# sungnyun/dualhyp

Hardware: AMD Instinct MI355X
Metric: corrected utterances/sec (TinyLlama-1.1B, 5+5 hyps, 512->64 tok) (higher is better)
Workload: dtype bf16; 1 GPU; DualHyp inference, TinyLlama-1.1B bf16 + LoRA r16 (q,k,v,proj), batch 32/GPU synthetic 5+5-hyp prompts, 512-token prompt -> 64 generated tokens, greedy; batch_per_gpu=32, parallelism=replicas x1, batches_in_flight_per_gpu=64, schedule=merged, decode_rows_per_launch=2048

## Files before the change

### dualhyp_amd/csrc/capi.hip

```cpp
#include "common.h"
#include "tuning.h"
#include <stdarg.h>

static thread_local char g_err[512] = "";

void dh_set_error(const char* fmt, ...) {
    va_list ap;
    va_start(ap, fmt);
    vsnprintf(g_err, sizeof(g_err), fmt, ap);
    va_end(ap);
}

extern "C" const char* dh_last_error(void) { return g_err; }
extern "C" int dh_abi_version(void) { return DH_ABI_VERSION; }

int dh_stop_pack(const char* name, const dh_stop_spec* stop, bool start_ok, dh_stop_args& out) {
    out = dh_stop_args{};
    if (!stop) return 0;
    DH_CHECK(stop->n_seqs >= 0 && stop->n_seqs <= DH_MAX_STOP_SEQS, "%s: %d stop sequences, at most %d are supported", name, stop->n_seqs,
             DH_MAX_STOP_SEQS);
    DH_CHECK(stop->n_seqs == 0 || (stop->seqs && stop->h_seq_len), "%s: %d stop sequences without their ids or their lengths", name,
             stop->n_seqs);
    uint32_t lens = 0;
    for (int i = 0; i < stop->n_seqs; ++i) {
// ... 10 lines not shown
    return 0;
}

int dh_nucleus_pack(const char* name, float top_p, float min_p, dh_nucleus_args& out) {
    out = dh_nucleus_args{};
    DH_CHECK(top_p > 0.f && top_p <= 1.f, "%s: top_p=%g is not in (0, 1] (1 = off)", name, (double)top_p);
    DH_CHECK(min_p >= 0.f && min_p <= 1.f, "%s: min_p=%g is not in [0, 1] (0 = off)", name, (double)min_p);
    out.top_p = top_p;
    out.min_p = min_p;
    out.min_p_on = min_p > 0.f;
    out.lmin = out.min_p_on ? (float)log((double)min_p) : 0.f;
    return 0;
}

int dh_penalty_pack(const char* name, const dh_penalty_args* in, dh_penalty_args& out) {
    out = DH_PENALTY_OFF;
    if (!in) return 0;
    DH_CHECK(in->repetition >= 0.125f && in->repetition <= 8.f, "%s: repetition=%g is not in [1/8, 8] (1 = off)", name, (double)in->repetition);
    DH_CHECK(in->frequency >= -8.f && in->frequency <= 8.f, "%s: frequency=%g is not in [-8, 8] (0 = off)", name, (double)in->frequency);
    DH_CHECK(in->presence >= -8.f && in->presence <= 8.f, "%s: presence=%g is not in [-8, 8] (0 = off)", name, (double)in->presence);
    out = *in;
    return 0;
}

extern "C" int dh_device_info(char* h_buf, int h_buf_len, int* h_num_cu, int64_t* h_hbm_bytes) {
    int n = 0;
    hipError_t e = hipGetDeviceCount(&n);
    DH_CHECK(e == hipSuccess && n > 0, "no HIP device visible (%s)", hipGetErrorString(e));
    int dev = 0;
    DH_HIP(hipGetDevice(&dev));
    hipDeviceProp_t p;
    DH_HIP(hipGetDeviceProperties(&p, dev));
    if (h_buf && h_buf_len > 0) {
        strncpy(h_buf, p.gcnArchName, h_buf_len - 1);
        h_buf[h_buf_len - 1] = 0;
    }
    if (h_num_cu) *h_num_cu = p.multiProcessorCount;
    if (h_hbm_bytes) *h_hbm_bytes = (int64_t)p.totalGlobalMem;
    return 0;
}

namespace {

enum Accept { ANY, BOOL , RANGE , ONE_OF  };
struct TuningRow { int key; int* knob; Accept accept; int a, b, c; };
constexpr int NO_MAX = 0x7fffffff;

const TuningRow TUNING[] = {
    {0, &g_skinny_variant, ANY, 0, 0, 0},
    {1, &g_gemm_variant, ANY, 0, 0, 0},
    {2, &g_swiglu2, ANY, 0, 0, 0},
    {3, &g_mid, ANY, 0, 0, 0},
    {4, &g_linear_phase, ANY, 0, 0, 0},
    {5, &g_gemm_gm, RANGE, 0, NO_MAX, 0},
    {6, &g_dt_min_rows, RANGE, 1, NO_MAX, 0},
    {7, &g_chain_min_rows, RANGE, 1, NO_MAX, 0},
    {8, &g_dt_stages, ANY, 0, 0, 0},
    {9, &g_gemm128_stages, ANY, 0, 0, 0},
    {10, &g_decode_tiled_rows, RANGE, 0, NO_MAX, 0},
    {11, &g_rows_ct, RANGE, 0, NO_MAX, 0},
    {12, &g_fuse_qkv_rope, ANY, 0, 0, 0},
    {13, &g_mid_wlds, ANY, 0, 0, 0},
    {14, &g_rows_ng, ONE_OF, 0, 8, 10},
    {15, &g_dt_wide, ANY, 0, 0, 0},
    {16, &g_short_kps, ONE_OF, 8, 16, 16},
    {17, &g_pairs_wn, ONE_OF, 0, 2, 4},
    {18, &g_pairs_min_rows, RANGE, 1, NO_MAX, 0},
    {19, &g_fp8_tile, ONE_OF, 0, 128, 256},
    {20, &g_fp8_gm, RANGE, 0, 64, 0},
    {21, &g_pairs_wt, BOOL, 0, 0, 0},
    {22, &g_w4_persist, RANGE, 0, 2, 0},
    {23, &g_prune_last_layer, BOOL, 0, 0, 0},
    {24, &g_w4_fast_epi, ANY, 0, 0, 0},
    {25, &g_w4_persist_qkv, BOOL, 0, 0, 0},
    {26, &g_tn_mfma, BOOL, 0, 0, 0},
    {27, &g_attn_bwd_dq_group, BOOL, 0, 0, 0},
    {28, &g_tail_split, BOOL, 0, 0, 0},
    {29, &g_attn_bwd_dkdv_img, BOOL, 0, 0, 0},
    {30, &g_w4_persist_lora, BOOL, 0, 0, 0},
    {31, &g_skinny_n, BOOL, 0, 0, 0},
    {40, &g_attn_chain, BOOL, 0, 0, 0},
    {41, &g_finish_hoist_rows, RANGE, -1, NO_MAX, 0},
    {42, &g_prefill_wpb, ONE_OF, 0, 2, 4},
};

}

extern "C" int dh_set_tuning(int key, int value) {
    for (const TuningRow& r : TUNING) {
        if (r.key != key) continue;
        if (r.accept == RANGE && (value < r.a || value > r.b)) break;
        if (r.accept == ONE_OF && value != r.a && value != r.b && value != r.c) break;
        *r.knob = r.accept == BOOL ? value != 0 : value;
        return 0;
    }
    dh_set_error("dh_set_tuning: unknown key %d", key);
    return 1;
}
```

### dualhyp_amd/csrc/decode_fused.hip

```cpp
#include "common.h"
#include "tuning.h"

int g_attn_chain = 1;
int g_finish_hoist_rows = -1;

#ifdef DH_ATTN_STAMPS
__device__ unsigned long long g_attn_stamps[4096 * 8];
#define ATTN_STAMP(i) do { if (threadIdx.x == 0 && blockIdx.x < 4096) g_attn_stamps[blockIdx.x * 8 + (i)] = __builtin_amdgcn_s_memrealtime(); } while (0)
#define ATTN_DRAIN() __builtin_amdgcn_s_waitcnt(0)
extern "C" int dh_debug_attn_stamps(unsigned long long* out) {
    return hipMemcpyFromSymbol(out, HIP_SYMBOL(g_attn_stamps), sizeof(g_attn_stamps)) == hipSuccess ? 0 : 1;
}
#else
#define ATTN_STAMP(i)
#define ATTN_DRAIN()
#endif

namespace {

constexpr int DCOLS = 16;
constexpr int MAXP = 16;

template <int HS, int PMAX, int NW>
__global__ __launch_bounds__(NW * 64, NW == 16 ? 1 : (NW == 6 ? 3 : (HS == 64 ? 4 : 2))) void attn_decode_fused_kernel(
    const float* __restrict__ qkv32, int n_part, int pairs, int n_seq, int ldq, int qkv_dim,
    const bf16_t* __restrict__ lora_b, float lora_scale, int split0, int split1,
    const bf16_t* __restrict__ cos, const bf16_t* __restrict__ sin, const int32_t* __restrict__ seq_slot,
    const int32_t* __restrict__ kv_len, bf16_t* __restrict__ k_cache, bf16_t* __restrict__ vT_cache,
    bf16_t* __restrict__ y, int n_head, int n_groups, int s_max, float scale) {
    constexpr int KS = HS / 16, DT = HS / 32, HALF = HS / 2;
    extern __shared__ __attribute__((aligned(16))) char smem[];
    const int pair = blockIdx.x, seq = pair / n_groups, g = pair % n_groups;
    const int q_per_kv = n_head / n_groups;
    const int tid = threadIdx.x, lane = tid & 63, wave = tid >> 6;
    const int lr = lane & 31, lh = lane >> 5;
    const int slot = seq_slot[seq];
    const int len = kv_len[seq], pos = len - 1;
    bf16_t* sQ = reinterpret_cast<bf16_t*>(smem);
    float* sKn = reinterpret_cast<float*>(smem + 16 * HS * 2);
    float* sVn = sKn + HS;
    float* sXa = sVn + HS;
    float* sSn = sXa + 48;
    float* sPm = sSn + 16;
    float* sPl = sPm + NW * DCOLS;
    float* sPo = sPl + NW * DCOLS;
    constexpr int NT_ = NW * 64;
    ATTN_STAMP(0);

    constexpr int PF = NW == 6 ? 2 : 1;
    struct VF { bf16x8 v; };
    struct Tile { bf16x8 kf[KS]; VF vf[DT][2]; };
    Tile tl[PF];
    const bf16_t* kbase = k_cache + ((size_t)slot * n_groups + g) * s_max * HS;
    const bf16_t* vbase = vT_cache + ((size_t)slot * n_groups + g) * HS * s_max;
    const int n_tiles = (pos + 31) / 32;
    auto load_tile = [&](Tile& T, int t) {
#pragma unroll
        for (int ks = 0; ks < KS; ++ks)
            T.kf[ks] = __builtin_nontemporal_load(reinterpret_cast<const bf16x8*>(kbase + kfrag_blk<HS>(t, ks) + lane * 8));
#pragma unroll
        for (int dt = 0; dt < DT; ++dt)
#pragma unroll
            for (int s2 = 0; s2 < 2; ++s2)
                T.vf[dt][s2].v = __builtin_nontemporal_load(reinterpret_cast<const bf16x8*>(vbase + vfrag_blk<HS>(t, dt, s2) + lane * 8));
    };
#pragma unroll
    for (int p = 0; p < PF; ++p)
        if (wave + NW * p < n_tiles) load_tile(tl[p], wave + NW * p);

    const float* row0 = qkv32 + (size_t)seq * ldq;
    const size_t pstride = (size_t)n_seq * ldq;
    auto psum = [&](int c) {
        float v[PMAX];
#pragma unroll
        for (int p = 0; p < PMAX; ++p) v[p] = p < n_part ? row0[p * pstride + c] : 0.f;
        float s = 0.f;
        if (pairs) {
#pragma unroll
            for (int p = 0; p < PMAX; p += 2) s += v[p] + v[p + 1];
        } else {
#pragma unroll
            for (int p = 0; p < PMAX; ++p) s += v[p];
        }
        return s;
    };
    if (lora_b != nullptr && tid < 48) sXa[tid] = rbf(psum(qkv_dim + tid));
    for (int i = tid; i < 16 * HS; i += NT_) sQ[i] = 0;
// ... 698 lines not shown
        const int c0 = (tid + i * 256) * 8;
        if (c0 < d) {
            float acc[8];
#pragma unroll
            for (int e = 0; e < 8; ++e) acc[e] = 0.f;
            for (int p0 = 0; p0 < n_part; p0 += 4) {
                float4 a0[4], a1[4];
#pragma unroll
                for (int q = 0; q < 4; ++q) {
                    if (HOIST && i == 0 && p0 == 0) {
                        a0[q] = ha0[q]; a1[q] = ha1[q];
                        continue;
                    }
                    const int p = p0 + q < n_part ? p0 + q : p0;
                    a0[q] = *reinterpret_cast<const float4*>(hrow + p * pstride + c0);
                    a1[q] = *reinterpret_cast<const float4*>(hrow + p * pstride + c0 + 4);
                }
                if (pairs) {
#pragma unroll
                    for (int q = 0; q < 4; q += 2) {
                        if (p0 + q < n_part) {
                            const bool two = p0 + q + 1 < n_part;
                            const float4 b0 = two ? a0[q + 1] : float4{0.f, 0.f, 0.f, 0.f}, b1 = two ? a1[q + 1] : float4{0.f, 0.f, 0.f, 0.f};
                            acc[0] += a0[q].x + b0.x; acc[1] += a0[q].y + b0.y; acc[2] += a0[q].z + b0.z; acc[3] += a0[q].w + b0.w;
                            acc[4] += a1[q].x + b1.x; acc[5] += a1[q].y + b1.y; acc[6] += a1[q].z + b1.z; acc[7] += a1[q].w + b1.w;
                        }
                    }
                } else {
#pragma unroll
                for (int q = 0; q < 4; ++q) {
                    if (p0 + q < n_part) {
                        acc[0] += a0[q].x; acc[1] += a0[q].y; acc[2] += a0[q].z; acc[3] += a0[q].w;
                        acc[4] += a1[q].x; acc[5] += a1[q].y; acc[6] += a1[q].z; acc[7] += a1[q].w;
                    }
                }
                }
            }
            const uint4 xr = HOIST && i == 0 ? hxr : *reinterpret_cast<const uint4*>(x_resid + (size_t)row * d + c0);
            const bf16_t* xp = reinterpret_cast<const bf16_t*>(&xr);
            uint4 xo;
            bf16_t* xop = reinterpret_cast<bf16_t*>(&xo);
#pragma unroll
            for (int e = 0; e < 8; ++e) {
                float o = rbf(acc[e]);
                if (lora_b != nullptr) {
                    const uint4* b4 = reinterpret_cast<const uint4*>(lora_b + (size_t)(c0 + e) * 16);
                    float l = 0.f;
#pragma unroll
                    for (int h = 0; h < 2; ++h) {
                        const uint4 bv = b4[h];
                        const bf16_t* bp = reinterpret_cast<const bf16_t*>(&bv);
#pragma unroll
                        for (int k = 0; k < 8; ++k) l = fmaf(sXa[h * 8 + k], bf2f(bp[k]), l);
                    }
                    o = rbf(o + rbf(rbf(l) * lora_scale));
                }
                xop[e] = f2bf(bf2f(xp[e]) + o);
                v[i][e] = bf2f(xop[e]);
                ss += rbf(v[i][e] * v[i][e]);
            }
            *reinterpret_cast<uint4*>(x_out + (size_t)row * d + c0) = xo;
        }
    }
    ss = wave_sum(ss);
    if (lane == 0) sRed[wave] = ss;
    __syncthreads();
    ss = sRed[0] + sRed[1] + sRed[2] + sRed[3];
    const float ms = rbf(ss / (float)d);
    const float t = rbf(ms + eps);
    const bool tail = row_tail != nullptr && row_tail[row] != 0;
    const float r = tail ? rbf(1.0f / rbf(sqrtf(t))) : rbf(1.0f / sqrtf(t));
#pragma unroll
    for (int i = 0; i < MAXC; ++i) {
        const int c0 = (tid + i * 256) * 8;
        if (c0 < d) {
            const uint4 wu = HOIST && i == 0 ? hwu : *reinterpret_cast<const uint4*>(w_norm + c0);
            const bf16_t* wp = reinterpret_cast<const bf16_t*>(&wu);
            uint4 o;
            bf16_t* op = reinterpret_cast<bf16_t*>(&o);
#pragma unroll
            for (int e = 0; e < 8; ++e) op[e] = f2bf(bf2f(wp[e]) * rbf(v[i][e] * r));
            *reinterpret_cast<uint4*>(xn_out + (size_t)row * d + c0) = o;
        }
    }
}

}

extern "C" int dh_attn_decode_fused_bf16(const float* qkv32, int n_part, int pairs, int n_seq, int qkv_dim, int n_ext,
                                         const dh_bf16* lora_b, float lora_scale, int split0, int split1,
                                         const dh_bf16* cos, const dh_bf16* sin, const int32_t* seq_slot,
                                         const int32_t* kv_len, dh_bf16* k_cache, dh_bf16* vT_cache, dh_bf16* y,
                                         int n_head, int n_groups, int hs, int s_max, void* stream) {
    DH_CHECK(qkv32 && cos && sin && seq_slot && kv_len && k_cache && vT_cache && y, "dh_attn_decode_fused_bf16: null argument");
    DH_CHECK(n_groups > 0 && n_head % n_groups == 0 && n_head / n_groups <= DCOLS, "dh_attn_decode_fused_bf16: bad head counts");
    DH_CHECK(hs == 64 || hs == 96 || hs == 128, "dh_attn_decode_fused_bf16: head_size %d unsupported", hs);
    DH_CHECK(s_max % 64 == 0 && n_part >= 1 && n_part <= MAXP, "dh_attn_decode_fused_bf16: bad s_max / n_part");
    DH_CHECK(qkv_dim == (n_head + 2 * n_groups) * hs, "dh_attn_decode_fused_bf16: qkv_dim mismatch");
    DH_CHECK(lora_b == nullptr || n_ext >= 48, "dh_attn_decode_fused_bf16: LoRA needs the 48 x·A^T columns");
    if (n_seq <= 0) return 0;
    const float scale = 1.0f / sqrtf((float)hs);
    hipStream_t s = (hipStream_t)stream;
    dim3 grid(n_seq * n_groups);
#define ATT_LAUNCH(HSV, PM)                                                                                           \
    hipLaunchKernelGGL((attn_decode_fused_kernel<HSV, PM, attn_fused_waves<HSV>()>), grid, dim3(64 * attn_fused_waves<HSV>()), attn_fused_lds<HSV>(), s, qkv32, n_part, pairs, n_seq,  \
                       qkv_dim + n_ext, qkv_dim, lora_b, lora_scale, split0, split1, cos, sin, seq_slot, kv_len, k_cache,  \
                       vT_cache, y, n_head, n_groups, s_max, scale)
#define CHAIN_LAUNCH(PM)                                                                                              \
    hipLaunchKernelGGL((attn_decode_chain_kernel<64, PM, CHAIN_NW>), grid, dim3(64 * CHAIN_NW), attn_chain_lds<64>(), s, qkv32, n_part, pairs, n_seq,  \
                       qkv_dim + n_ext, qkv_dim, lora_b, lora_scale, split0, split1, cos, sin, seq_slot, kv_len, k_cache,  \
                       vT_cache, y, n_head, n_groups, s_max, scale)
    if (hs == 64) {
        DH_MAX_LDS_ONCE((attn_decode_fused_kernel<64, 2, attn_fused_waves<64>()>), attn_fused_lds<64>());
        DH_MAX_LDS_ONCE((attn_decode_fused_kernel<64, 8, attn_fused_waves<64>()>), attn_fused_lds<64>());
        DH_MAX_LDS_ONCE((attn_decode_fused_kernel<64, 16, attn_fused_waves<64>()>), attn_fused_lds<64>());
        const bool chain = g_attn_chain != 0 && attn_fused_waves<64>() == CHAIN_NW && (n_head / n_groups + 1) * 32 + 64 <= 64 * CHAIN_NW;
        if (chain) {
            DH_MAX_LDS_ONCE((attn_decode_chain_kernel<64, 2, CHAIN_NW>), attn_chain_lds<64>());
            DH_MAX_LDS_ONCE((attn_decode_chain_kernel<64, 8, CHAIN_NW>), attn_chain_lds<64>());
            DH_MAX_LDS_ONCE((attn_decode_chain_kernel<64, 16, CHAIN_NW>), attn_chain_lds<64>());
            if (n_part <= 2) CHAIN_LAUNCH(2);
            else if (n_part <= 8) CHAIN_LAUNCH(8);
            else CHAIN_LAUNCH(16);
        } else if (n_part <= 2) ATT_LAUNCH(64, 2);
        else if (n_part <= 8) ATT_LAUNCH(64, 8);
        else ATT_LAUNCH(64, 16);
    } else if (hs == 96) {
        DH_MAX_LDS_ONCE((attn_decode_fused_kernel<96, 2, 8>), attn_fused_lds<96>());
        DH_MAX_LDS_ONCE((attn_decode_fused_kernel<96, 8, 8>), attn_fused_lds<96>());
        DH_MAX_LDS_ONCE((attn_decode_fused_kernel<96, 16, 8>), attn_fused_lds<96>());
        if (n_part <= 2) ATT_LAUNCH(96, 2);
        else if (n_part <= 8) ATT_LAUNCH(96, 8);
        else ATT_LAUNCH(96, 16);
    } else {
        DH_MAX_LDS_ONCE((attn_decode_fused_kernel<128, 2, 8>), attn_fused_lds<128>());
        DH_MAX_LDS_ONCE((attn_decode_fused_kernel<128, 8, 8>), attn_fused_lds<128>());
        DH_MAX_LDS_ONCE((attn_decode_fused_kernel<128, 16, 8>), attn_fused_lds<128>());
        if (n_part <= 2) ATT_LAUNCH(128, 2);
        else if (n_part <= 8) ATT_LAUNCH(128, 8);
        else ATT_LAUNCH(128, 16);
    }
#undef ATT_LAUNCH
#undef CHAIN_LAUNCH
    DH_LAUNCH_CHECK();
    return 0;
}

int dh_attn_verify_fused_impl(const float* qkv32, int n_part, int pairs, int n_seq, int S, int qkv_dim, int n_ext,
                              const dh_bf16* lora_b, float lora_scale, int split0, int split1, const dh_bf16* cos,
                              const dh_bf16* sin, const int32_t* seq_slot, const int32_t* kv_len, dh_bf16* k_cache,
                              dh_bf16* vT_cache, dh_bf16* y, int n_head, int n_groups, int hs, int s_max, int p_max, void* stream) {
    DH_CHECK(qkv32 && cos && sin && seq_slot && kv_len && k_cache && vT_cache && y, "attn_verify_fused: null argument");
    DH_CHECK(n_groups > 0 && n_head % n_groups == 0, "attn_verify_fused: bad head counts");
    DH_CHECK(S >= 2 && S <= 8, "attn_verify_fused: S = %d positions per sequence, 2 .. 8 are served", S);
    DH_CHECK(S * (n_head / n_groups) <= 32, "attn_verify_fused: %d positions x %d heads per group exceed 32 query columns",
             S, n_head / n_groups);
    DH_CHECK(hs == 64 || hs == 96 || hs == 128, "attn_verify_fused: head_size %d unsupported", hs);
    DH_CHECK(s_max % 64 == 0 && p_max > 0 && p_max <= s_max && n_part >= 1 && n_part <= MAXP, "attn_verify_fused: bad s_max / p_max / n_part");
    DH_CHECK(qkv_dim == (n_head + 2 * n_groups) * hs, "attn_verify_fused: qkv_dim mismatch");
    DH_CHECK(lora_b == nullptr || n_ext >= 48, "attn_verify_fused: LoRA needs the 48 x·A^T columns");
    if (n_seq <= 0) return 0;
    const float scale = 1.0f / sqrtf((float)hs);
    hipStream_t s = (hipStream_t)stream;
    dim3 grid(n_seq * n_groups);
    const int ncol = S * (n_head / n_groups);
#define VER_LAUNCH(HSV, PM)                                                                                           \
    hipLaunchKernelGGL((attn_verify_fused_kernel<HSV, PM, attn_fused_waves<HSV>()>), grid, dim3(64 * attn_fused_waves<HSV>()), attn_verify_lds<HSV>(S, ncol), s, qkv32, n_part, pairs, \
                       n_seq * S, qkv_dim + n_ext, qkv_dim, lora_b, lora_scale, split0, split1, cos, sin, seq_slot, kv_len, k_cache,  \
                       vT_cache, y, n_head, n_groups, s_max, p_max, S, scale)
#define VER_HS(HSV)                                                                                                   \
    do {                                                                                                              \
        DH_MAX_LDS_ONCE((attn_verify_fused_kernel<HSV, 2, attn_fused_waves<HSV>()>), attn_verify_lds<HSV>(8, 32));    \
        DH_MAX_LDS_ONCE((attn_verify_fused_kernel<HSV, 8, attn_fused_waves<HSV>()>), attn_verify_lds<HSV>(8, 32));    \
        DH_MAX_LDS_ONCE((attn_verify_fused_kernel<HSV, 16, attn_fused_waves<HSV>()>), attn_verify_lds<HSV>(8, 32));   \
        if (n_part <= 2) VER_LAUNCH(HSV, 2);                                                                          \
        else if (n_part <= 8) VER_LAUNCH(HSV, 8);                                                                     \
        else VER_LAUNCH(HSV, 16);                                                                                     \
    } while (0)
    if (hs == 64) VER_HS(64);
    else if (hs == 96) VER_HS(96);
    else VER_HS(128);
#undef VER_HS
#undef VER_LAUNCH
    DH_LAUNCH_CHECK();
    return 0;
}

extern "C" int dh_attn_verify_fused_bf16(const float* qkv32, int n_part, int pairs, int n_seq, int S, int qkv_dim, int n_ext,
                                         const dh_bf16* lora_b, float lora_scale, int split0, int split1, const dh_bf16* cos,
                                         const dh_bf16* sin, const int32_t* seq_slot, const int32_t* kv_len, dh_bf16* k_cache,
                                         dh_bf16* vT_cache, dh_bf16* y, int n_head, int n_groups, int hs, int s_max, int p_max,
                                         void* stream) {
    return dh_attn_verify_fused_impl(qkv32, n_part, pairs, n_seq, S, qkv_dim, n_ext, lora_b, lora_scale, split0, split1, cos, sin,
                                     seq_slot, kv_len, k_cache, vT_cache, y, n_head, n_groups, hs, s_max, p_max, stream);
}

constexpr int FINISH_HOIST_ROWS = 128;

extern "C" int dh_finish_norm_bf16(const float* h32, int n_part, int pairs, int rows, int d, int n_ext, const dh_bf16* lora_b,
                                   float lora_scale, const dh_bf16* x_resid, const dh_bf16* w_norm, dh_bf16* x_out,
                                   dh_bf16* xn_out, float eps, const uint8_t* row_tail, void* stream) {
    DH_CHECK(h32 && x_resid && w_norm && x_out && xn_out, "dh_finish_norm_bf16: null argument");
    DH_CHECK(d % 8 == 0 && d <= 8192 && n_part >= 1 && n_part <= MAXP, "dh_finish_norm_bf16: unsupported d=%d", d);
    DH_CHECK(lora_b == nullptr || n_ext >= 16, "dh_finish_norm_bf16: LoRA needs the 16 x·A^T columns");
    DH_CHECK((d + n_ext) % 4 == 0, "dh_finish_norm_bf16: row stride must be a multiple of 4 floats");
    if (rows <= 0) return 0;
    hipStream_t s = (hipStream_t)stream;
    dim3 grid(rows), block(256);
    const int ldh = d + n_ext;
#define LAUNCH(MAXC) do {                                                                                             \
        if (hoist) hipLaunchKernelGGL((finish_norm_kernel<MAXC, true>), grid, block, 0, s, h32, n_part, pairs, rows, ldh, lora_b,  \
                                      lora_scale, x_resid, w_norm, x_out, xn_out, d, eps, row_tail);                  \
        else hipLaunchKernelGGL((finish_norm_kernel<MAXC, false>), grid, block, 0, s, h32, n_part, pairs, rows, ldh, lora_b,       \
                                lora_scale, x_resid, w_norm, x_out, xn_out, d, eps, row_tail);                        \
    } while (0)
    const int hoist_rows = g_finish_hoist_rows >= 0 ? g_finish_hoist_rows : FINISH_HOIST_ROWS;
    const bool hoist = hoist_rows > 0 && rows >= hoist_rows;
    if (d <= 2048) { LAUNCH(1); }
    else if (d <= 4096) { LAUNCH(2); }
    else { LAUNCH(4); }
#undef LAUNCH
    DH_LAUNCH_CHECK();
    return 0;
}
```

### dualhyp_amd/csrc/gemm_dt.hip

```cpp
#include "common.h"
#include "gemm.h"

int g_dt_stages = 0;
int g_dt_wide = 0;

namespace {

constexpr int TB = 128;
constexpr int BKD = 64;
template <int WN> constexpr int stage_bytes() { return (WN * 64 + TB) * BKD * 2; }

__device__ __forceinline__ int swz7(int row) { return (row >> 1) & 7; }

struct DtArgs {
    const bf16_t* x;
    const bf16_t* w;
    const bf16_t* w2;
    void* y;
    const bf16_t* vec_a;
    const bf16_t* vec_b;
    const bf16_t* resid;
    int M, N, K, n_main, seg;
    int split_kt;
    int wt;
};

template <int MODE, int NSTAGE, int WN = 2>
__global__ __launch_bounds__(WN * 128) void gemm_dt_kernel(DtArgs a) {
    constexpr int STAGE = stage_bytes<WN>();
    constexpr int ASZ = WN * 64 * BKD * 2;
    constexpr int NB = 16 / (2 * WN);
    constexpr int PER = 4 + NB;
    extern __shared__ __attribute__((aligned(16))) char smem[];
    const int tid = threadIdx.x, lane = tid & 63, wave = tid >> 6;
    const int wn = wave >> 1, wm = wave & 1;
    const int frow = lane & 15, kg = lane >> 4;
    const int m_tiles = (a.M + TB - 1) / TB;
    int tile, ky = 0;
    {
        const int nwg = gridDim.x * gridDim.y, bid = blockIdx.x + gridDim.x * blockIdx.y, xcd = bid & 7, q = nwg >> 3, r = nwg & 7;
        tile = (xcd < r ? xcd * (q + 1) : r * (q + 1) + (xcd - r) * q) + (bid >> 3);
        if (MODE == 4) { ky = tile / (int)gridDim.x; tile -= ky * (int)gridDim.x; }
    }
    const int tm = tile % m_tiles, tn = tile / m_tiles;
    const int m0 = tm * TB;
    const int n0 = MODE == 1 ? tn * (WN * 32) : tn * (WN * 64);

    const bf16_t* srcA[4];
    const bf16_t* srcB[NB];
#pragma unroll
    for (int j = 0; j < 4; ++j) {
        const int R = wave * 4 + j;
        const int row = R * 8 + (lane >> 3);
        const int chunk = (lane & 7) ^ swz7(row);
        const bf16_t* base = a.w;
        int n;
        if (MODE == 1) {
            const int half = (row >> 5) & 1;
            n = n0 + (row >> 6) * 32 + (row & 31);
            n = n < a.N ? n : a.N - 1;
            base = half ? a.w2 : a.w;
        } else {
            n = n0 + row;
            n = n < a.N ? n : a.N - 1;
            if ((MODE == 0 || MODE == 4) && n >= a.n_main) { base = a.w2; n -= a.n_main; }
        }
        srcA[j] = base + (size_t)n * a.K + chunk * 8 + (MODE == 4 ? (size_t)ky * a.split_kt * BKD : 0);
    }
#pragma unroll
    for (int j = 0; j < NB; ++j) {
        const int R = wave * NB + j;
        const int row = R * 8 + (lane >> 3);
        const int chunk = (lane & 7) ^ swz7(row);
        int m = m0 + row;
        m = m < a.M ? m : a.M - 1;
        srcB[j] = a.x + (size_t)m * a.K + chunk * 8 + (MODE == 4 ? (size_t)ky * a.split_kt * BKD : 0);
    }
    auto stage = [&](int kt) __attribute__((always_inline)) {
        char* sA = smem + (kt % NSTAGE) * STAGE;
        char* sB = sA + ASZ;
#pragma unroll
        for (int j = 0; j < 4; ++j) glds16(srcA[j] + kt * BKD, sA + (wave * 4 + j) * 1024);
#pragma unroll
        for (int j = 0; j < NB; ++j) glds16(srcB[j] + kt * BKD, sB + (wave * NB + j) * 1024);
    };
    auto wait_next = [&](int ahead) __attribute__((always_inline)) {
        if (NSTAGE >= 4 && ahead >= 2) asm volatile("s_waitcnt vmcnt(%0)" ::"n"(2 * PER) : "memory");
        else if (NSTAGE >= 3 && ahead >= 1) asm volatile("s_waitcnt vmcnt(%0)" ::"n"(PER) : "memory");
        else asm volatile("s_waitcnt vmcnt(0)" ::: "memory");
    };

    f32x4 cur[4][4], tot[4][4];
#pragma unroll
    for (int i = 0; i < 4; ++i)
#pragma unroll
        for (int j = 0; j < 4; ++j) {
            cur[i][j] = f32x4{0.f, 0.f, 0.f, 0.f};
            tot[i][j] = f32x4{0.f, 0.f, 0.f, 0.f};
        }
    const int sw = swz7(frow);
    const int offA = (wn * 64 + frow) * 128, offB = (wm * 64 + frow) * 128;
    const int nk = MODE == 4 ? min(a.split_kt, a.K / BKD - ky * a.split_kt) : a.K / BKD;
    const int seg_kt = a.seg / 2;
    f32x4 pairacc[MODE == 0 ? 4 : 1][MODE == 0 ? 4 : 1];
    int seg_idx = 0;

    auto fold_segment = [&](bool last) __attribute__((always_inline)) {
        if (MODE == 0) {
            const bool second = seg_idx & 1;
#pragma unroll
            for (int i = 0; i < 4; ++i)
#pragma unroll
                for (int j = 0; j < 4; ++j) {
                    if (second) tot[i][j] += pairacc[i][j] + cur[i][j];
                    else if (last) tot[i][j] += cur[i][j];
                    else pairacc[i][j] = cur[i][j];
                    cur[i][j] = f32x4{0.f, 0.f, 0.f, 0.f};
                }
            ++seg_idx;
        } else {
#pragma unroll
            for (int i = 0; i < 4; ++i)
#pragma unroll
                for (int j = 0; j < 4; ++j) {
                    tot[i][j] += cur[i][j];
                    cur[i][j] = f32x4{0.f, 0.f, 0.f, 0.f};
                }
        }
    };
    int in_seg = 0;
    if constexpr (WN == 4 && NSTAGE == 3) {
    auto stage_w = [&](int kt) __attribute__((always_inline)) {
        char* sA = smem + (kt % NSTAGE) * STAGE;
#pragma unroll
        for (int j = 0; j < 4; ++j) glds16(srcA[j] + kt * BKD, sA + (wave * 4 + j) * 1024);
    };
    auto stage_x = [&](int kt) __attribute__((always_inline)) {
        char* sB = smem + (kt % NSTAGE) * STAGE + ASZ;
#pragma unroll
        for (int j = 0; j < NB; ++j) glds16(srcB[j] + kt * BKD, sB + (wave * NB + j) * 1024);
    };
    auto read_frags = [&](int kt, int ks, bf16x8 (&fa)[4], bf16x8 (&fb)[4]) __attribute__((always_inline)) {
        const char* sA = smem + (kt % NSTAGE) * STAGE;
        const char* sB = sA + ASZ;
        const int co = ((ks * 4 + kg) ^ sw) << 4;
#pragma unroll
        for (int i = 0; i < 4; ++i) {
            fa[i] = *reinterpret_cast<const bf16x8*>(sA + offA + i * 2048 + co);
            fb[i] = *reinterpret_cast<const bf16x8*>(sB + offB + i * 2048 + co);
        }
    };
    auto mma = [&](const bf16x8 (&fa)[4], const bf16x8 (&fb)[4]) __attribute__((always_inline)) {
#pragma unroll
        for (int i = 0; i < 4; ++i)
#pragma unroll
            for (int j = 0; j < 4; ++j) cur[i][j] = __builtin_amdgcn_mfma_f32_16x16x32_bf16(fa[i], fb[j], cur[i][j], 0, 0, 0);
    };
    stage(0);
    if (1 < nk) stage(1);
    if (2 < nk) stage_w(2);
    if (2 < nk) asm volatile("s_waitcnt vmcnt(%0)" ::"n"(PER + 4) : "memory");
    else if (1 < nk) asm volatile("s_waitcnt vmcnt(%0)" ::"n"(PER) : "memory");
    else asm volatile("s_waitcnt vmcnt(0)" ::: "memory");
    __builtin_amdgcn_s_barrier();
    bf16x8 fa0[4], fb0[4], fa1[4], fb1[4];
    read_frags(0, 0, fa0, fb0);
    for (int kt = 0; kt < nk; ++kt) {
        read_frags(kt, 1, fa1, fb1);
        if (kt + 2 < nk) stage_x(kt + 2);
        mma(fa0, fb0);
        asm volatile("s_waitcnt lgkmcnt(0)" ::: "memory");
        if (kt + 2 < nk) asm volatile("s_waitcnt vmcnt(%0)" ::"n"(PER) : "memory");
        else asm volatile("s_waitcnt vmcnt(0)" ::: "memory");
        __builtin_amdgcn_s_barrier();
        if (kt + 1 < nk) read_frags(kt + 1, 0, fa0, fb0);
        if (kt + 3 < nk) stage_w(kt + 3);
        mma(fa1, fb1);
        if (++in_seg == seg_kt || kt + 1 == nk) {
            in_seg = 0;
            fold_segment(kt + 1 == nk);
        }
    }
    } else {
#pragma unroll
    for (int p = 0; p < NSTAGE - 1; ++p)
        if (p < nk) stage(p);
    wait_next((nk < NSTAGE - 1 ? nk : NSTAGE - 1) - 1);
    __builtin_amdgcn_s_barrier();
    for (int kt = 0; kt < nk; ++kt) {
        const bool pre = kt + NSTAGE - 1 < nk;
        const char* sA = smem + (kt % NSTAGE) * STAGE;
        const char* sB = sA + ASZ;
        if (pre) stage(kt + NSTAGE - 1);
#pragma unroll
        for (int ks = 0; ks < 2; ++ks) {
            const int co = ((ks * 4 + kg) ^ sw) << 4;
            bf16x8 fa[4], fb[4];
#pragma unroll
            for (int i = 0; i < 4; ++i) {
                fa[i] = *reinterpret_cast<const bf16x8*>(sA + offA + i * 2048 + co);
                fb[i] = *reinterpret_cast<const bf16x8*>(sB + offB + i * 2048 + co);
            }
#pragma unroll
            for (int i = 0; i < 4; ++i)
#pragma unroll
                for (int j = 0; j < 4; ++j)
                    cur[i][j] = __builtin_amdgcn_mfma_f32_16x16x32_bf16(fa[i], fb[j], cur[i][j], 0, 0, 0);
        }
        if (++in_seg == seg_kt || kt + 1 == nk) {
            in_seg = 0;
            fold_segment(kt + 1 == nk);
        }
        {
            const int issued = (kt + NSTAGE - 1 < nk ? kt + NSTAGE - 1 : nk - 1);
            wait_next(issued - (kt + 1));
        }
        __builtin_amdgcn_s_barrier();
    }
    }

#pragma unroll
    for (int j = 0; j < 4; ++j) {
        const int m = m0 + wm * 64 + j * 16 + frow;
        if (m >= a.M) continue;
        if (MODE == 1) {
#pragma unroll
            for (int i = 0; i < 2; ++i) {
                const int n = n0 + wn * 32 + i * 16 + kg * 4;
                if (n >= a.N) continue;
                float o[4];
#pragma unroll
                for (int r = 0; r < 4; ++r) {
                    const float gt = rbf(tot[i][j][r]), up = rbf(tot[i + 2][j][r]);
                    o[r] = rbf(silu_fast(gt)) * up;
                }
                *reinterpret_cast<uint2*>((bf16_t*)a.y + (size_t)m * a.N + n) = make_uint2(pack2bf(o[0], o[1]), pack2bf(o[2], o[3]));
            }
        } else {
#pragma unroll
            for (int i = 0; i < 4; ++i) {
                const int n = n0 + wn * 64 + i * 16 + kg * 4;
                if (n >= a.N) continue;
                if (MODE == 0 || MODE == 4) {
                    float* yo = (float*)a.y + (MODE == 4 ? (size_t)ky * a.M * a.N : 0);
                    float* dst = yo + (size_t)m * a.N + n;
                    if (MODE == 4 && a.wt) asm volatile("global_store_dwordx4 %0, %1, off sc1" ::"v"(dst), "v"(tot[i][j]) : "memory");
                    else *reinterpret_cast<f32x4*>(dst) = tot[i][j];
                    continue;
                }
                float o[4];
#pragma unroll
                for (int r = 0; r < 4; ++r) {
                    o[r] = rbf(tot[i][j][r]);
                    if (MODE == 2) o[r] = rbf(bf2f(a.vec_a[n + r]) * rbf(o[r] + bf2f(a.vec_b[n + r])));
                }
                if (MODE == 3 && a.resid != nullptr) {
                    const uint2 rv = *reinterpret_cast<const uint2*>(a.resid + (size_t)m * a.N + n);
                    const bf16_t* rp = reinterpret_cast<const bf16_t*>(&rv);
#pragma unroll
                    for (int r = 0; r < 4; ++r) o[r] = bf2f(rp[r]) + o[r];
                }
                *reinterpret_cast<uint2*>((bf16_t*)a.y + (size_t)m * a.N + n) = make_uint2(pack2bf(o[0], o[1]), pack2bf(o[2], o[3]));
            }
        }
    }
}

template <int MODE, int NSTAGE, int WN = 2>
int launch_dt_n(const DtArgs& a, int blocks, hipStream_t s, int ny = 1) {
    constexpr int lds = NSTAGE * stage_bytes<WN>();
    DH_MAX_LDS_ONCE((gemm_dt_kernel<MODE, NSTAGE, WN>), lds);
    dh_gemm_route(MODE == 0 ? DH_ROUTE_CHAIN_TILED : MODE == 4 ? DH_ROUTE_PAIRS_TILED : DH_ROUTE_DT_FUSED);
    hipLaunchKernelGGL((gemm_dt_kernel<MODE, NSTAGE, WN>), dim3(blocks, ny), dim3(WN * 128), lds, s, a);
    DH_LAUNCH_CHECK();
    return 0;
}

template <int MODE>
int launch_dt(const DtArgs& a, hipStream_t s) {
    const int m_tiles = cdiv(a.M, TB);
    if ((MODE == 1 || MODE == 2) && (g_dt_wide ? g_dt_wide > 0 : a.M >= 256))
        return launch_dt_n<MODE == 2 ? 2 : 1, 3, 4>(a, m_tiles * cdiv(a.N, MODE == 1 ? 128 : 256), s);
    const int n_tiles = cdiv(a.N, MODE == 1 ? 64 : TB);
    const int blocks = m_tiles * n_tiles;
    const int stages = g_dt_stages ? g_dt_stages : (blocks > 256 ? 2 : 4);
    return stages == 2 ? launch_dt_n<MODE, 2>(a, blocks, s) : launch_dt_n<MODE, 4>(a, blocks, s);
}

}

int g_dt_min_rows = 129;
int g_chain_min_rows = 1 << 30;

int dh_chain_tiled(const bf16_t* x, const bf16_t* w, const bf16_t* w_ext, float* y32, int M, int n_main, int n_ext, int K,
                   int kps, hipStream_t s) {
    DtArgs a{x, w, w_ext ? w_ext : w, y32, nullptr, nullptr, nullptr, M, n_main + n_ext, K, n_main, kps, 0, 0};
    return launch_dt<0>(a, s);
}

int g_pairs_wn = 0;
int g_pairs_wt = 0;
int dh_pairs_tiled(const bf16_t* x, const bf16_t* w, const bf16_t* w_ext, float* y32, int M, int n_main, int n_ext, int K,
                   int kps, hipStream_t s) {
    const int N = n_main + n_ext, nslices = cdiv(K / 32, kps), ny = (nslices + 1) / 2;
    DtArgs a{x, w, w_ext ? w_ext : w, y32, nullptr, nullptr, nullptr, M, N, K, n_main, kps, kps, g_pairs_wt};
    const int m_tiles = cdiv(M, TB);
    const int wide_blocks = m_tiles * cdiv(N, 256) * ny;
    const bool wide = g_pairs_wn ? g_pairs_wn == 4 : wide_blocks >= 160;
    if (wide) return launch_dt_n<4, 3, 4>(a, m_tiles * cdiv(N, 256), s, ny);
    const int blocks = m_tiles * cdiv(N, TB);
    return blocks * ny > 256 ? launch_dt_n<4, 2>(a, blocks, s, ny) : launch_dt_n<4, 4>(a, blocks, s, ny);
}

bool dh_linear_dt_ok(const GemmArgs& a, int epilogue, int seg) {
    return a.M >= (epilogue == DH_EPI_ADAPTER ? (g_dt_min_rows < 65 ? g_dt_min_rows : 65) : g_dt_min_rows) && a.M > 64 && a.K % BKD == 0 && seg > 0 && seg % 2 == 0 && (a.K / 32) % seg == 0 && a.N % 4 == 0 &&
           (epilogue == DH_EPI_PLAIN || epilogue == DH_EPI_SWIGLU || epilogue == DH_EPI_ADAPTER);
}

int dh_linear_dt(const GemmArgs& g, int epilogue, int seg, hipStream_t s) {
    DtArgs a{g.x, g.w, g.w2, g.y, g.vec_a, g.vec_b, g.resid, g.M, g.N, g.K, g.N, seg, 0, 0};
    switch (epilogue) {
        case DH_EPI_SWIGLU: return launch_dt<1>(a, s);
        case DH_EPI_ADAPTER: return launch_dt<2>(a, s);
        case DH_EPI_PLAIN: return launch_dt<3>(a, s);
    }
    dh_set_error("dh_linear_dt: unsupported epilogue %d", epilogue);
    return 1;
}
```

### dualhyp_amd/csrc/tuning.h

```cpp
#pragma once

extern int g_gemm128_stages, g_gemm_variant, g_tail_split, g_linear_phase;
extern int g_gemm_gm, g_w4_persist, g_w4_fast_epi, g_w4_persist_qkv, g_w4_persist_lora;
extern int g_mid, g_mid_wlds;
extern int g_dt_stages, g_dt_wide, g_dt_min_rows, g_chain_min_rows, g_pairs_wn, g_pairs_wt;
extern int g_pairs_min_rows, g_skinny_n;
__attribute__((visibility("hidden"))) extern int g_skinny_variant, g_swiglu2, g_rows_ct, g_rows_ng;
extern int g_fp8_tile, g_fp8_gm;
extern int g_decode_tiled_rows, g_short_kps, g_fuse_qkv_rope, g_prune_last_layer;
extern int g_attn_bwd_dkdv_img, g_attn_bwd_dq_group;
extern int g_tn_mfma;
extern int g_attn_chain, g_finish_hoist_rows;
extern int g_prefill_wpb;
```

Baseline: 821.7 utterances/s.

## Add multi-row finish-norm kernel and 8-wave chain GEMM with 32x64 wave tiles

Adds a finish_norm_rows kernel in which each block handles several rows (default 4) once there are at least 2048 rows. It prefetches the next row's partial sums and residual, and loads the LoRA-B and norm weights once per block rather than once per row. It also adds a chain-GEMM variant that uses 512 threads with 32x64 wave tiles, and lowers the chain-tiled threshold from effectively never to 1536 rows, so the tiled chain path now runs at large decode batches. Risks are higher register pressure, lower occupancy, and a different reduction order in the new routes.

```diff
diff --git a/dualhyp_amd/csrc/capi.hip b/dualhyp_amd/csrc/capi.hip
--- a/dualhyp_amd/csrc/capi.hip
+++ b/dualhyp_amd/csrc/capi.hip
@@ -116,6 +116,8 @@
     {40, &g_attn_chain, BOOL, 0, 0, 0},
     {41, &g_finish_hoist_rows, RANGE, -1, NO_MAX, 0},
     {42, &g_prefill_wpb, ONE_OF, 0, 2, 4},
+    {43, &g_finish_rows_min, RANGE, -1, NO_MAX, 0},
+    {44, &g_finish_rpb, RANGE, 0, 64, 0},
 };
 
 }
diff --git a/dualhyp_amd/csrc/decode_fused.hip b/dualhyp_amd/csrc/decode_fused.hip
--- a/dualhyp_amd/csrc/decode_fused.hip
+++ b/dualhyp_amd/csrc/decode_fused.hip
@@ -3,6 +3,8 @@
 
 int g_attn_chain = 1;
 int g_finish_hoist_rows = -1;
+int g_finish_rows_min = -1;
+int g_finish_rpb = 0;
 
 #ifdef DH_ATTN_STAMPS
 __device__ unsigned long long g_attn_stamps[4096 * 8];
@@ -867,6 +869,174 @@
             for (int e = 0; e < 8; ++e) op[e] = f2bf(bf2f(wp[e]) * rbf(v[i][e] * r));
             *reinterpret_cast<uint4*>(xn_out + (size_t)row * d + c0) = o;
         }
+    }
+}
+
+template <int MAXC, int PF, int XP, bool LORA>
+__global__ __launch_bounds__(256) void finish_norm_rows_kernel(const float* __restrict__ h32, int n_part, int pairs, int rows, int ldh,
+                                                               const bf16_t* __restrict__ lora_b, float lora_scale,
+                                                               const bf16_t* __restrict__ x_resid,
+                                                               const bf16_t* __restrict__ w_norm, bf16_t* __restrict__ x_out,
+                                                               bf16_t* __restrict__ xn_out, int d, float eps,
+                                                               const uint8_t* __restrict__ row_tail, int rpb) {
+    __shared__ float sXa[2][16];
+    __shared__ float sRed[2][4];
+    const int tid = threadIdx.x, lane = tid & 63, wave = tid >> 6;
+    const int row0 = blockIdx.x * rpb, nrow = min(rpb, rows - row0);
+    const size_t pstride = (size_t)rows * ldh;
+    const bool own = tid * 8 < d;
+    struct Pre { float xa[XP]; float4 a0[PF], a1[PF]; uint4 xr; };
+    auto request = [&](Pre& P, int row) __attribute__((always_inline)) {
+        const float* hrow = h32 + (size_t)row * ldh;
+        if (LORA && tid < 16) {
+#pragma unroll
+            for (int p = 0; p < XP; ++p) P.xa[p] = p < n_part ? hrow[p * pstride + d + tid] : 0.f;
+        }
+        if (own) {
+            const int c0 = tid * 8;
+#pragma unroll
+            for (int q = 0; q < PF; ++q) {
+                const int p = q < n_part ? q : 0;
+                P.a0[q] = *reinterpret_cast<const float4*>(hrow + p * pstride + c0);
+                P.a1[q] = *reinterpret_cast<const float4*>(hrow + p * pstride + c0 + 4);
+            }
+            P.xr = *reinterpret_cast<const uint4*>(x_resid + (size_t)row * d + c0);
+        }
+    };
+    auto xa_sum = [&](const Pre& P) __attribute__((always_inline)) {
+        float s = 0.f;
+        if (pairs) {
+#pragma unroll
+            for (int p = 0; p < XP; p += 2) s += P.xa[p] + (p + 1 < XP ? P.xa[p + 1] : 0.f);
+        } else {
+#pragma unroll
+            for (int p = 0; p < XP; ++p) s += P.xa[p];
+        }
+        return rbf(s);
+    };
+    auto add_group = [&](float (&acc)[8], const float4* a0, const float4* a1, int p0, auto G_) __attribute__((always_inline)) {
+        constexpr int G = decltype(G_)::value;
+        if (pairs) {
+#pragma unroll
+            for (int q = 0; q < G; q += 2) {
+                if (p0 + q < n_part) {
+                    const bool two = q + 1 < G && p0 + q + 1 < n_part;
+                    const float4 b0 = two ? a0[q + 1 < G ? q + 1 : q] : float4{0.f, 0.f, 0.f, 0.f}, b1 = two ? a1[q + 1 < G ? q + 1 : q] : float4{0.f, 0.f, 0.f, 0.f};
+                    acc[0] += a0[q].x + b0.x; acc[1] += a0[q].y + b0.y; acc[2] += a0[q].z + b0.z; acc[3] += a0[q].w + b0.w;
+                    acc[4] += a1[q].x + b1.x; acc[5] += a1[q].y + b1.y; acc[6] += a1[q].z + b1.z; acc[7] += a1[q].w + b1.w;
+                }
+            }
+        } else {
+#pragma unroll
+            for (int q = 0; q < G; ++q) {
+                if (p0 + q < n_part) {
+                    acc[0] += a0[q].x; acc[1] += a0[q].y; acc[2] += a0[q].z; acc[3] += a0[q].w;
+                    acc[4] += a1[q].x; acc[5] += a1[q].y; acc[6] += a1[q].z; acc[7] += a1[q].w;
+                }
+            }
+        }
+    };
+
+    Pre pa, pb;
+    request(pa, row0);
+    if (nrow > 1) request(pb, row0 + 1);
+    uint4 bq[LORA ? 8 : 1][2];
+    uint4 hwu = {};
+    if (own) {
+        if (LORA) {
+#pragma unroll
+            for (int e = 0; e < 8; ++e) {
+                const uint4* b4 = reinterpret_cast<const uint4*>(lora_b + (size_t)(tid * 8 + e) * 16);
+                bq[e][0] = b4[0];
+                bq[e][1] = b4[1];
+            }
+        }
+        hwu = *reinterpret_cast<const uint4*>(w_norm + tid * 8);
+    }
+    if (LORA && tid < 16) sXa[0][tid] = xa_sum(pa);
+    asm volatile("s_waitcnt lgkmcnt(0)" ::: "memory");
+    __builtin_amdgcn_s_barrier();
+    asm volatile("" ::: "memory");
+
+    auto do_row = [&](Pre& P, Pre& Q, int k) __attribute__((always_inline)) {
+        const int row = row0 + k, par = k & 1;
+        const float* hrow = h32 + (size_t)row * ldh;
+        const bool tail = row_tail != nullptr && row_tail[row] != 0;
+        float v[MAXC][8];
+        float ss = 0.f;
+#pragma unroll
+        for (int i = 0; i < MAXC; ++i) {
+            const int c0 = (tid + i * 256) * 8;
+            if (c0 < d) {
+                float acc[8];
+#pragma unroll
+                for (int e = 0; e < 8; ++e) acc[e] = 0.f;
+                if (i == 0) add_group(acc, P.a0, P.a1, 0, std::integral_constant<int, PF>{});
+                for (int p0 = i == 0 ? PF : 0; p0 < n_part; p0 += 4) {
+                    float4 a0[4], a1[4];
+#pragma unroll
+                    for (int q = 0; q < 4; ++q) {
+                        const int p = p0 + q < n_part ? p0 + q : p0;
+                        a0[q] = *reinterpret_cast<const float4*>(hrow + p * pstride + c0);
+                        a1[q] = *reinterpret_cast<const float4*>(hrow + p * pstride + c0 + 4);
+                    }
+                    add_group(acc, a0, a1, p0, std::integral_constant<int, 4>{});
+                }
+                const uint4 xr = i == 0 ? P.xr : *reinterpret_cast<const uint4*>(x_resid + (size_t)row * d + c0);
+                const bf16_t* xp = reinterpret_cast<const bf16_t*>(&xr);
+                uint4 xo;
+                bf16_t* xop = reinterpret_cast<bf16_t*>(&xo);
+#pragma unroll
+                for (int e = 0; e < 8; ++e) {
+                    float o = rbf(acc[e]);
+                    if (LORA) {
+                        const uint4* b4 = reinterpret_cast<const uint4*>(lora_b + (size_t)(c0 + e) * 16);
+                        float l = 0.f;
+#pragma unroll
+                        for (int h = 0; h < 2; ++h) {
+                            uint4 bv = i == 0 ? bq[e][h] : b4[h];
+                            if (i == 0) asm volatile("" : "+v"(bv.x), "+v"(bv.y), "+v"(bv.z), "+v"(bv.w));
+                            const bf16_t* bp = reinterpret_cast<const bf16_t*>(&bv);
+#pragma unroll
+                            for (int kk = 0; kk < 8; ++kk) l = fmaf(sXa[par][h * 8 + kk], bf2f(bp[kk]), l);
+                        }
+                        o = rbf(o + rbf(rbf(l) * lora_scale));
+                    }
+                    xop[e] = f2bf(bf2f(xp[e]) + o);
+                    v[i][e] = bf2f(xop[e]);
+                    ss += rbf(v[i][e] * v[i][e]);
+                }
+                *reinterpret_cast<uint4*>(x_out + (size_t)row * d + c0) = xo;
+            }
+        }
+        if (k + 2 < nrow) request(P, row + 2);
+        ss = wave_sum(ss);
+        if (lane == 0) sRed[par][wave] = ss;
+        if (LORA && k + 1 < nrow && tid < 16) sXa[par ^ 1][tid] = xa_sum(Q);
+        asm volatile("s_waitcnt lgkmcnt(0)" ::: "memory");
+        __builtin_amdgcn_s_barrier();
+        asm volatile("" ::: "memory");
+        ss = sRed[par][0] + sRed[par][1] + sRed[par][2] + sRed[par][3];
+        const float ms = rbf(ss / (float)d);
+        const float t = rbf(ms + eps);
+        const float r = tail ? rbf(1.0f / rbf(sqrtf(t))) : rbf(1.0f / sqrtf(t));
+#pragma unroll
+        for (int i = 0; i < MAXC; ++i) {
+            const int c0 = (tid + i * 256) * 8;
+            if (c0 < d) {
+                const uint4 wu = i == 0 ? hwu : *reinterpret_cast<const uint4*>(w_norm + c0);
+                const bf16_t* wp = reinterpret_cast<const bf16_t*>(&wu);
+                uint4 o;
+                bf16_t* op = reinterpret_cast<bf16_t*>(&o);
+#pragma unroll
+                for (int e = 0; e < 8; ++e) op[e] = f2bf(bf2f(wp[e]) * rbf(v[i][e] * r));
+                *reinterpret_cast<uint4*>(xn_out + (size_t)row * d + c0) = o;
+            }
+        }
+    };
+    for (int k = 0; k < nrow; k += 2) {
+        do_row(pa, pb, k);
+        if (k + 1 < nrow) do_row(pb, pa, k + 1);
     }
 }
 
@@ -981,6 +1151,8 @@
 }
 
 constexpr int FINISH_HOIST_ROWS = 128;
+constexpr int FINISH_ROWS_MIN = 2048;
+constexpr int FINISH_RPB = 4;
 
 extern "C" int dh_finish_norm_bf16(const float* h32, int n_part, int pairs, int rows, int d, int n_ext, const dh_bf16* lora_b,
                                    float lora_scale, const dh_bf16* x_resid, const dh_bf16* w_norm, dh_bf16* x_out,
@@ -999,6 +1171,30 @@
         else hipLaunchKernelGGL((finish_norm_kernel<MAXC, false>), grid, block, 0, s, h32, n_part, pairs, rows, ldh, lora_b,       \
                                 lora_scale, x_resid, w_norm, x_out, xn_out, d, eps, row_tail);                        \
     } while (0)
+    const int multi_rows = g_finish_rows_min >= 0 ? g_finish_rows_min : FINISH_ROWS_MIN;
+    if (multi_rows > 0 && rows >= multi_rows) {
+        const int rpb = g_finish_rpb > 0 ? g_finish_rpb : FINISH_RPB;
+        dim3 mgrid((rows + rpb - 1) / rpb);
+#define LAUNCH_ROWS(MAXC, PF, XP, LORA)                                                                                  \
+        hipLaunchKernelGGL((finish_norm_rows_kernel<MAXC, PF, XP, LORA>), mgrid, block, 0, s, h32, n_part, pairs, rows, ldh, lora_b,  \
+                           lora_scale, x_resid, w_norm, x_out, xn_out, d, eps, row_tail, rpb)
+#define LAUNCH_MAXC(MAXC) do {                                                                                        \
+        if (lora_b != nullptr) {                                                                                      \
+            if (n_part <= 1) LAUNCH_ROWS(MAXC, 1, 1, true);                                                           \
+            else if (n_part <= 4) LAUNCH_ROWS(MAXC, 4, 4, true);                                                      \
+            else LAUNCH_ROWS(MAXC, 4, MAXP, true);                                                                    \
+        } else if (n_part <= 1) LAUNCH_ROWS(MAXC, 1, 1, false);                                                       \
+        else if (n_part <= 4) LAUNCH_ROWS(MAXC, 4, 1, false);                                                         \
+        else LAUNCH_ROWS(MAXC, 8, 1, false);                                                                          \
+    } while (0)
+        if (d <= 2048) LAUNCH_MAXC(1);
+        else if (d <= 4096) LAUNCH_MAXC(2);
+        else LAUNCH_MAXC(4);
+#undef LAUNCH_MAXC
+#undef LAUNCH_ROWS
+        DH_LAUNCH_CHECK();
+        return 0;
+    }
     const int hoist_rows = g_finish_hoist_rows >= 0 ? g_finish_hoist_rows : FINISH_HOIST_ROWS;
     const bool hoist = hoist_rows > 0 && rows >= hoist_rows;
     if (d <= 2048) { LAUNCH(1); }
diff --git a/dualhyp_amd/csrc/gemm_dt.hip b/dualhyp_amd/csrc/gemm_dt.hip
--- a/dualhyp_amd/csrc/gemm_dt.hip
+++ b/dualhyp_amd/csrc/gemm_dt.hip
@@ -25,14 +25,18 @@
     int wt;
 };
 
-template <int MODE, int NSTAGE, int WN = 2>
-__global__ __launch_bounds__(WN * 128) void gemm_dt_kernel(DtArgs a) {
+template <int MODE, int NSTAGE, int WN, int WI>
+__device__ __forceinline__ void gemm_dt_body(const DtArgs& a) {
+    static_assert(WI == 4 || (WI == 2 && MODE == 0 && !(WN == 4 && NSTAGE == 3)), "the 32 x 64 wave tile serves MODE 0 on the plain ring");
     constexpr int STAGE = stage_bytes<WN>();
     constexpr int ASZ = WN * 64 * BKD * 2;
-    constexpr int NB = 16 / (2 * WN);
-    constexpr int PER = 4 + NB;
+    constexpr int NWV = WN * 8 / WI;
+    constexpr int NA = WI;
+    constexpr int NB = 16 / NWV;
+    constexpr int PER = NA + NB;
     extern __shared__ __attribute__((aligned(16))) char smem[];
-    const int tid = threadIdx.x, lane = tid & 63, wave = tid >> 6;
+    const int tid = threadIdx.x, lane = tid & 63;
+    const int wave = WI == 2 ? __builtin_amdgcn_readfirstlane(tid >> 6) : tid >> 6;
     const int wn = wave >> 1, wm = wave & 1;
     const int frow = lane & 15, kg = lane >> 4;
     const int m_tiles = (a.M + TB - 1) / TB;
@@ -46,11 +50,11 @@
     const int m0 = tm * TB;
     const int n0 = MODE == 1 ? tn * (WN * 32) : tn * (WN * 64);
 
-    const bf16_t* srcA[4];
+    const bf16_t* srcA[NA];
     const bf16_t* srcB[NB];
 #pragma unroll
-    for (int j = 0; j < 4; ++j) {
-        const int R = wave * 4 + j;
+    for (int j = 0; j < NA; ++j) {
+        const int R = wave * NA + j;
         const int row = R * 8 + (lane >> 3);
         const int chunk = (lane & 7) ^ swz7(row);
         const bf16_t* base = a.w;
@@ -80,7 +84,7 @@
         char* sA = smem + (kt % NSTAGE) * STAGE;
         char* sB = sA + ASZ;
 #pragma unroll
-        for (int j = 0; j < 4; ++j) glds16(srcA[j] + kt * BKD, sA + (wave * 4 + j) * 1024);
+        for (int j = 0; j < NA; ++j) glds16(srcA[j] + kt * BKD, sA + (wave * NA + j) * 1024);
 #pragma unroll
         for (int j = 0; j < NB; ++j) glds16(srcB[j] + kt * BKD, sB + (wave * NB + j) * 1024);
     };
@@ -90,26 +94,26 @@
         else asm volatile("s_waitcnt vmcnt(0)" ::: "memory");
     };
 
-    f32x4 cur[4][4], tot[4][4];
-#pragma unroll
-    for (int i = 0; i < 4; ++i)
+    f32x4 cur[WI][4], tot[WI][4];
+#pragma unroll
+    for (int i = 0; i < WI; ++i)
 #pragma unroll
         for (int j = 0; j < 4; ++j) {
             cur[i][j] = f32x4{0.f, 0.f, 0.f, 0.f};
             tot[i][j] = f32x4{0.f, 0.f, 0.f, 0.f};
         }
     const int sw = swz7(frow);
-    const int offA = (wn * 64 + frow) * 128, offB = (wm * 64 + frow) * 128;
+    const int offA = (wn * (WI * 16) + frow) * 128, offB = (wm * 64 + frow) * 128;
     const int nk = MODE == 4 ? min(a.split_kt, a.K / BKD - ky * a.split_kt) : a.K / BKD;
     const int seg_kt = a.seg / 2;
-    f32x4 pairacc[MODE == 0 ? 4 : 1][MODE == 0 ? 4 : 1];
+    f32x4 pairacc[MODE == 0 ? WI : 1][MODE == 0 ? 4 : 1];
     int seg_idx = 0;
 
     auto fold_segment = [&](bool last) __attribute__((always_inline)) {
         if (MODE == 0) {
             const bool second = seg_idx & 1;
 #pragma unroll
-            for (int i = 0; i < 4; ++i)
+            for (int i = 0; i < WI; ++i)
 #pragma unroll
                 for (int j = 0; j < 4; ++j) {
                     if (second) tot[i][j] += pairacc[i][j] + cur[i][j];
@@ -120,7 +124,7 @@
             ++seg_idx;
         } else {
 #pragma unroll
-            for (int i = 0; i < 4; ++i)
+            for (int i = 0; i < WI; ++i)
 #pragma unroll
                 for (int j = 0; j < 4; ++j) {
                     tot[i][j] += cur[i][j];
@@ -195,6 +199,17 @@
 #pragma unroll
         for (int ks = 0; ks < 2; ++ks) {
             const int co = ((ks * 4 + kg) ^ sw) << 4;
+            if constexpr (WI == 2) {
+                bf16x8 fa[2];
+#pragma unroll
+                for (int i = 0; i < 2; ++i) fa[i] = *reinterpret_cast<const bf16x8*>(sA + offA + i * 2048 + co);
+#pragma unroll
+                for (int j = 0; j < 4; ++j) {
+                    const bf16x8 fb = *reinterpret_cast<const bf16x8*>(sB + offB + j * 2048 + co);
+#pragma unroll
+                    for (int i = 0; i < 2; ++i) cur[i][j] = __builtin_amdgcn_mfma_f32_16x16x32_bf16(fa[i], fb, cur[i][j], 0, 0, 0);
+                }
+            } else {
             bf16x8 fa[4], fb[4];
 #pragma unroll
             for (int i = 0; i < 4; ++i) {
@@ -206,6 +221,7 @@
 #pragma unroll
                 for (int j = 0; j < 4; ++j)
                     cur[i][j] = __builtin_amdgcn_mfma_f32_16x16x32_bf16(fa[i], fb[j], cur[i][j], 0, 0, 0);
+            }
         }
         if (++in_seg == seg_kt || kt + 1 == nk) {
             in_seg = 0;
@@ -223,7 +239,7 @@
     for (int j = 0; j < 4; ++j) {
         const int m = m0 + wm * 64 + j * 16 + frow;
         if (m >= a.M) continue;
-        if (MODE == 1) {
+        if constexpr (MODE == 1) {
 #pragma unroll
             for (int i = 0; i < 2; ++i) {
                 const int n = n0 + wn * 32 + i * 16 + kg * 4;
@@ -238,8 +254,8 @@
             }
         } else {
 #pragma unroll
-            for (int i = 0; i < 4; ++i) {
-                const int n = n0 + wn * 64 + i * 16 + kg * 4;
+            for (int i = 0; i < WI; ++i) {
+                const int n = n0 + wn * (WI * 16) + i * 16 + kg * 4;
                 if (n >= a.N) continue;
                 if (MODE == 0 || MODE == 4) {
                     float* yo = (float*)a.y + (MODE == 4 ? (size_t)ky * a.M * a.N : 0);
@@ -264,6 +280,22 @@
             }
         }
     }
+}
+
+template <int MODE, int NSTAGE, int WN = 2>
+__global__ __launch_bounds__(WN * 128) void gemm_dt_kernel(DtArgs a) { gemm_dt_body<MODE, NSTAGE, WN, 4>(a); }
+
+template <int NSTAGE>
+__global__ __launch_bounds__(512, NSTAGE == 2 ? 4 : 2) void gemm_dt_chain_kernel(DtArgs a) { gemm_dt_body<0, NSTAGE, 2, 2>(a); }
+
+template <int NSTAGE>
+int launch_chain_n(const DtArgs& a, int blocks, hipStream_t s) {
+    constexpr int lds = NSTAGE * stage_bytes<2>();
+    DH_MAX_LDS_ONCE((gemm_dt_chain_kernel<NSTAGE>), lds);
+    dh_gemm_route(DH_ROUTE_CHAIN_TILED);
+    hipLaunchKernelGGL((gemm_dt_chain_kernel<NSTAGE>), dim3(blocks), dim3(512), lds, s, a);
+    DH_LAUNCH_CHECK();
+    return 0;
 }
 
 template <int MODE, int NSTAGE, int WN = 2>
@@ -290,12 +322,14 @@
 }
 
 int g_dt_min_rows = 129;
-int g_chain_min_rows = 1 << 30;
+int g_chain_min_rows = 1536;
 
 int dh_chain_tiled(const bf16_t* x, const bf16_t* w, const bf16_t* w_ext, float* y32, int M, int n_main, int n_ext, int K,
                    int kps, hipStream_t s) {
     DtArgs a{x, w, w_ext ? w_ext : w, y32, nullptr, nullptr, nullptr, M, n_main + n_ext, K, n_main, kps, 0, 0};
-    return launch_dt<0>(a, s);
+    const int blocks = cdiv(M, TB) * cdiv(a.N, TB);
+    const int stages = g_dt_stages ? g_dt_stages : (blocks > 256 ? 2 : 4);
+    return stages == 2 ? launch_chain_n<2>(a, blocks, s) : launch_chain_n<4>(a, blocks, s);
 }
 
 int g_pairs_wn = 0;
diff --git a/dualhyp_amd/csrc/tuning.h b/dualhyp_amd/csrc/tuning.h
--- a/dualhyp_amd/csrc/tuning.h
+++ b/dualhyp_amd/csrc/tuning.h
@@ -10,5 +10,5 @@
 extern int g_decode_tiled_rows, g_short_kps, g_fuse_qkv_rope, g_prune_last_layer;
 extern int g_attn_bwd_dkdv_img, g_attn_bwd_dq_group;
 extern int g_tn_mfma;
-extern int g_attn_chain, g_finish_hoist_rows;
+extern int g_attn_chain, g_finish_hoist_rows, g_finish_rows_min, g_finish_rpb;
 extern int g_prefill_wpb;
```

Measured after the change: 846.1 utterances/s (median of 6 runs). 3.0% higher.
